# arbobendik/web-ray-tracer

Hardware: AMD Instinct MI355X
Metric: Mray/s at 1080p (spp x bounces x pixels / s) (higher is better)
Workload: dtype f32

## Files before the change

### web-ray-tracer_amd/csrc/flx_device.h

```cpp
#ifndef FLX_DEVICE_H
#define FLX_DEVICE_H

#include <hip/hip_runtime.h>
#include <stdint.h>

#include "flx_math.h"

#define FLX_DEV __device__ __forceinline__

namespace flx {

constexpr float PHI = 1.61803398874989484820459f;
constexpr float SQRT3 = 1.7320508075688772f;
constexpr float INV_PI = 0.3183098861837907f;
constexpr float INV_256 = 0.00390625f;
constexpr float INV_255 = 0.00392156862745098f;
constexpr float PI_F = 3.141592653589793f;
constexpr float BIAS = FLX_BIAS;
constexpr float POW32 = FLX_POW32;
constexpr float NEAR_VIEW_DEPTH = 0.5f;

struct f3 { float x, y, z; };
struct f4 { float x, y, z, w; };
struct M3 { f3 c0, c1, c2; };
// ... 555 lines not shown


FLX_DEV float divByRecip(float a, float d, float y) {
  float q = a * y;
  float r = __builtin_fmaf(-q, d, a);
  q = __builtin_fmaf(r, y, q);
  r = __builtin_fmaf(-q, d, a);
  return __builtin_fmaf(r, y, q);
}
FLX_DEV void reciprocalOfDir(const DeviceScene &sc, f3 d, f3 o, f3 &inv, bool &fast) {
  inv = F3(recipFast(d.x), recipFast(d.y), recipFast(d.z));
  const float LO = 8.673617379884035e-19f, HI = 1.152921504606847e18f, OHI = 5.764607523034235e17f;
  const float ax = flx_abs(d.x), ay = flx_abs(d.y), az = flx_abs(d.z);
  fast = sc.walk_fast_boxes != 0u && ax >= LO && ax <= HI && ay >= LO && ay <= HI && az >= LO && az <= HI &&
         flx_abs(o.x) <= OHI && flx_abs(o.y) <= OHI && flx_abs(o.z) <= OHI;
}
#ifndef FLX_WF_RECIP_DIV
#define FLX_WF_RECIP_DIV 1
#endif
FLX_DEV void walkPrepareRay(const DeviceScene &sc, WalkState &w) {
#if !FLX_WF_RECIP_DIV
  (void)sc; (void)w;
  return;
#endif
  reciprocalOfDir(sc, w.tR.dir, w.tR.origin, w.inv, w.fastDiv);
}
FLX_DEV bool rayCuboidRecip(float l, const WalkState &w, f3 minCorner, f3 maxCorner);
FLX_DEV bool rayCuboidR(float l, const WalkState &w, f3 minCorner, f3 maxCorner) {
#if !FLX_WF_RECIP_DIV
  return rayCuboid(l, w.tR, minCorner, maxCorner);
#else
  return rayCuboidRecip(l, w, minCorner, maxCorner);
#endif
}
FLX_DEV bool rayCuboidRecip(float l, const WalkState &w, f3 minCorner, f3 maxCorner) {
  const f3 o = w.tR.origin, d = w.tR.dir, y = w.inv;
  const f3 a0 = minCorner - o, a1 = maxCorner - o;
  uint32_t m = (flx_f2u(a0.x) << 1) - 2u;
  uint32_t t;
  t = (flx_f2u(a0.y) << 1) - 2u; m = t < m ? t : m;
  t = (flx_f2u(a0.z) << 1) - 2u; m = t < m ? t : m;
  t = (flx_f2u(a1.x) << 1) - 2u; m = t < m ? t : m;
  t = (flx_f2u(a1.y) << 1) - 2u; m = t < m ? t : m;
  t = (flx_f2u(a1.z) << 1) - 2u; m = t < m ? t : m;
  const bool aOk = m >= (0x2b800000u << 1) - 2u;
  f3 v0, v1;
  float tmin, tmax;
  if ((w.fastDiv && aOk)) {
    v0 = F3(divByRecip(a0.x, d.x, y.x), divByRecip(a0.y, d.y, y.y), divByRecip(a0.z, d.z, y.z));
    v1 = F3(divByRecip(a1.x, d.x, y.x), divByRecip(a1.y, d.y, y.y), divByRecip(a1.z, d.z, y.z));
    tmin = __builtin_fmaxf(__builtin_fmaxf(__builtin_fminf(v0.x, v1.x), __builtin_fminf(v0.y, v1.y)), __builtin_fminf(v0.z, v1.z));
    tmax = __builtin_fminf(__builtin_fminf(__builtin_fmaxf(v0.x, v1.x), __builtin_fmaxf(v0.y, v1.y)), __builtin_fmaxf(v0.z, v1.z));
    return tmax >= __builtin_fmaxf(tmin, BIAS) && tmin < l;
  }
  v0 = a0 / d;
  v1 = a1 / d;
  tmin = flx_max(flx_max(flx_min(v0.x, v1.x), flx_min(v0.y, v1.y)), flx_min(v0.z, v1.z));
  tmax = flx_min(flx_min(flx_max(v0.x, v1.x), flx_max(v0.y, v1.y)), flx_max(v0.z, v1.z));
  return tmax >= flx_max(tmin, BIAS) && tmin < l;
}

template <bool THICK = false> FLX_DEV bool rayCuboidFast(float l, const WalkState &w, f3 lo, f3 hi);
FLX_DEV Hit primaryWalkT(const DeviceScene &sc, const Ray &ray, float viewDepthPerS, uint32_t &visits) {
  Hit hit; hit.suv = F3(0.0f, 0.0f, 0.0f); hit.transformId = 0; hit.triangleId = -1;
  WalkState w;
  w.tR = ray; w.minLen = POW32;
  reciprocalOfDir(sc, ray.dir, ray.origin, w.inv, w.fastDiv);
  int cachedTI = 0;
  uint32_t link = sc.walk_root;
  while (link != WALK_END) {
    const size_t i = (size_t)linkIndex(link) * 3u;
    const float4 e0 = sc.walk[i], e1 = sc.walk[i + 1], e2 = sc.walk[i + 2];
    visits++;
    const int meta = __float_as_int(e2.z);
    if ((meta & 3) == 0) break;
    const int tI = (meta >> 2) << 1;
    if (tI != cachedTI) {
      const int iI = tI + 1;
      const M3 rotationII = rotation_at(sc, iI);
      cachedTI = tI;
      w.tR.origin = mul(rotationII, ray.origin + shift_at(sc, iI));
      w.tR.dir = mul(rotationII, ray.dir);
      reciprocalOfDir(sc, w.tR.dir, w.tR.origin, w.inv, w.fastDiv);
    }
    if ((meta & 3) == 1) {
      link = (uint32_t)__float_as_int(rayCuboidFast(w.minLen, w, F3(e0.x, e0.y, e0.z), F3(e0.w, e1.x, e1.y)) ? e2.x : e2.y);
    } else {
      f3 suv;
      if (moellerTrumborePrimaryE(F3(e0.x, e0.y, e0.z), F3(e0.w, e1.x, e1.y), F3(e1.z, e1.w, e2.x), w.tR, w.minLen, viewDepthPerS, suv)) {
        hit.suv = suv; hit.transformId = tI; hit.triangleId = __float_as_int(e2.w);
        w.minLen = suv.x;
      }
      link = (uint32_t)__float_as_int(e2.y);
    }
  }
  return hit;
}

typedef float flx_v4f_ __attribute__((ext_vector_type(4)));
extern "C" __device__ unsigned int __ockl_wfred_min_u32(unsigned int);
#ifndef FLX_PRIMARY_PREFETCH
#define FLX_PRIMARY_PREFETCH 0
#endif
#ifndef FLX_PRIMARY_LOCK_MIN
#define FLX_PRIMARY_LOCK_MIN 12
#endif
typedef __attribute__((address_space(4))) const flx_v4f_ fwd_cf4;
FLX_DEV void primaryVisit(const DeviceScene &sc, const Ray &ray, float viewDepthPerS, WalkState &w, int &cachedTI, Hit &hit, uint32_t &nxt,
                          float4 e0, float4 e1, float4 e2, int xfBase = 0 ) {
  const int meta = __float_as_int(e2.z);
  if ((meta & 3) == 0) { nxt = WALK_END; return; }
  const int tI = (meta >> 2) << 1;
  if (tI != cachedTI) {
    const int iI = tI + 1 + xfBase;
    const M3 rotationII = rotation_at(sc, iI);
    cachedTI = tI;
    w.tR.origin = mul(rotationII, ray.origin + shift_at(sc, iI));
    w.tR.dir = mul(rotationII, ray.dir);
    reciprocalOfDir(sc, w.tR.dir, w.tR.origin, w.inv, w.fastDiv);
  }
  if ((meta & 3) == 1) {
    nxt = (uint32_t)__float_as_int(rayCuboidFast(w.minLen, w, F3(e0.x, e0.y, e0.z), F3(e0.w, e1.x, e1.y)) ? e2.x : e2.y);
  } else {
    f3 suv;
    if (moellerTrumborePrimaryE(F3(e0.x, e0.y, e0.z), F3(e0.w, e1.x, e1.y), F3(e1.z, e1.w, e2.x), w.tR, w.minLen, viewDepthPerS, suv)) {
      hit.suv = suv; hit.transformId = tI; hit.triangleId = __float_as_int(e2.w);
      w.minLen = suv.x;
    }
    nxt = (uint32_t)__float_as_int(e2.y);
  }
}
FLX_DEV Hit primaryWalkF(const DeviceScene &sc, bool active, const Ray &ray, float viewDepthPerS, uint32_t &visits, int xfBase = 0) {
  Hit hit; hit.suv = F3(0.0f, 0.0f, 0.0f); hit.transformId = 0; hit.triangleId = -1;
  WalkState w;
  w.tR = ray; w.minLen = POW32;
  reciprocalOfDir(sc, ray.dir, ray.origin, w.inv, w.fastDiv);
  int cachedTI = 0;
  uint32_t nxt = active ? sc.fwd_root : WALK_END;
  const fwd_cf4 *L = (const fwd_cf4 *)sc.fwd;
  uint32_t thin = 0;
  for (;;) {
    const uint32_t i = __builtin_amdgcn_readfirstlane(__ockl_wfred_min_u32(nxt));
    if (i == WALK_END) return hit;
    uint32_t iu = i;
    asm volatile("" : "+s"(iu));
    const fwd_cf4 *E = L + (size_t)iu * 3u;
    const flx_v4f_ a = E[0], b = E[1], c = E[2];
    const bool mine = nxt == i;
    if (mine) {
      visits++;
      primaryVisit(sc, ray, viewDepthPerS, w, cachedTI, hit, nxt, make_float4(a.x, a.y, a.z, a.w), make_float4(b.x, b.y, b.z, b.w), make_float4(c.x, c.y, c.z, c.w), xfBase);
    }
    thin = (uint32_t)__popcll(flx_ballot(mine)) < (uint32_t)FLX_PRIMARY_LOCK_MIN ? thin + 1u : 0u;
    if (thin >= 2u) break;
  }
#if FLX_PRIMARY_PREFETCH
  if (nxt != WALK_END) {
    size_t i = (size_t)nxt * 3u;
    float4 e0 = sc.fwd[i], e1 = sc.fwd[i + 1], e2 = sc.fwd[i + 2];
    while (nxt != WALK_END) {
      const int meta = __float_as_int(e2.z);
      const bool box = (meta & 3) == 1;
      const uint32_t linkA = (uint32_t)__float_as_int(box ? e2.x : e2.y), linkB = (uint32_t)__float_as_int(e2.y);
      const size_t ia = (size_t)((meta & 3) == 0 || linkA == WALK_END ? 0u : linkA) * 3u, ib = (size_t)((meta & 3) == 0 || linkB == WALK_END ? 0u : linkB) * 3u;
      const float4 a0 = sc.fwd[ia], a1 = sc.fwd[ia + 1], a2 = sc.fwd[ia + 2];
      float4 b0 = a0, b1 = a1, b2 = a2;
      if (box) { b0 = sc.fwd[ib]; b1 = sc.fwd[ib + 1]; b2 = sc.fwd[ib + 2]; }
      visits++;
      primaryVisit(sc, ray, viewDepthPerS, w, cachedTI, hit, nxt, e0, e1, e2);
      const bool tookA = nxt == linkA;
      e0 = tookA ? a0 : b0; e1 = tookA ? a1 : b1; e2 = tookA ? a2 : b2;
    }
  }
#else
  while (nxt != WALK_END) {
    const size_t i = (size_t)nxt * 3u;
    const float4 e0 = sc.fwd[i], e1 = sc.fwd[i + 1], e2 = sc.fwd[i + 2];
    visits++;
    primaryVisit(sc, ray, viewDepthPerS, w, cachedTI, hit, nxt, e0, e1, e2, xfBase);
  }
#endif
  return hit;
}

template <bool COUNT>
FLX_DEV bool walkFetchT(const DeviceScene &sc, const float4 *lds, uint32_t ldsCount, WalkState &w, WalkEntry &cur, WorkCounters &cnt) {
  if ((uint32_t)w.i == WALK_END) return true;
  const uint32_t i = linkIndex((uint32_t)w.i);
  if (i < ldsCount) { cur.e0 = lds[3 * i]; cur.e1 = lds[3 * i + 1]; cur.e2 = lds[3 * i + 2]; }
  else { cur.e0 = sc.walk[3 * (size_t)i]; cur.e1 = sc.walk[3 * (size_t)i + 1]; cur.e2 = sc.walk[3 * (size_t)i + 2]; }
  if (COUNT) { if (w.mode == 0) cnt.shadow_visits++; else cnt.closest_visits++; }
  const int meta = __float_as_int(cur.e2.z);
  int tI = (meta >> 2) << 1;
  if (tI != w.cachedTI) {
    int iI = tI + 1;
    M3 rotationII = rotation_at(sc, iI);
    w.cachedTI = tI;
    w.tR.origin = mul(rotationII, w.src.origin + shift_at(sc, iI));
    f3 d = mul(rotationII, w.src.dir);
    w.tR.dir = (w.mode == 0) ? normalize(d) : d;
    walkPrepareRay(sc, w);
  }
  return (meta & 3) == 0;
}
FLX_DEV bool walkIsBoxT(const WalkEntry &cur) { return (__float_as_int(cur.e2.z) & 3) == 1; }
FLX_DEV bool walkIsBoxL(const WalkState &w) { return linkKind((uint32_t)w.i) == 1u; }
FLX_DEV void walkBoxT(WalkState &w, const WalkEntry &cur) {
  const bool hit = rayCuboidR(w.minLen, w, F3(cur.e0.x, cur.e0.y, cur.e0.z), F3(cur.e0.w, cur.e1.x, cur.e1.y));
  w.i = hit ? __float_as_int(cur.e2.x) : __float_as_int(cur.e2.y);
}
#ifndef FLX_MT_BRANCHFREE
#define FLX_MT_BRANCHFREE 1
#endif
FLX_DEV bool moellerTrumboreAny(f3 a, f3 edge1, f3 edge2, const Ray &ray, float l, bool cull, f3 &suv) {
  f3 pvec = cross(ray.dir, edge2);
  float det = dot(edge1, pvec);
  bool detBad = cull ? (det < BIAS) : (flx_abs(det) < BIAS);
  float inv_det = recipOfDet(det, detBad);
  f3 tvec = ray.origin - a;
  float u = dot(tvec, pvec) * inv_det;
  f3 qvec = cross(tvec, edge1);
  float v = dot(ray.dir, qvec) * inv_det;
  float uvSum = u + v;
  float s = dot(edge2, qvec) * inv_det;
  bool uBad = (u < BIAS) || (u > 1.0f);
  bool vBad = (v < BIAS) || (uvSum > 1.0f);
#if FLX_MT_BRANCHFREE
  const bool sLe = (s <= l) | (!cull & __builtin_isunordered(s, l));
  const bool sGt = (s > BIAS) | (!cull & (s != s));
  const bool sOk = sLe & sGt;
  suv = F3(s, u, v);
  return !detBad & !uBad & !vBad & sOk;
#else
  bool sOk = cull ? ((s <= l) && (s > BIAS)) : (!(s > l) && !(s <= BIAS));
  suv = F3(s, u, v);
  return !detBad && !uBad && !vBad && sOk;
#endif
}
#ifndef FLX_WF_LINK_XFORM
#define FLX_WF_LINK_XFORM 1
#endif
#ifndef FLX_WF_LINK_KIND
#define FLX_WF_LINK_KIND 1
#endif
#ifndef FLX_WF_LINK_ISBOX
#define FLX_WF_LINK_ISBOX 1
#endif
#ifndef FLX_WF_FLAT_FETCH
#define FLX_WF_FLAT_FETCH 1
#endif
FLX_DEV bool walkTriT(WalkState &w, const WalkEntry &cur) {
  f3 a = F3(cur.e0.x, cur.e0.y, cur.e0.z), edge1 = F3(cur.e0.w, cur.e1.x, cur.e1.y), edge2 = F3(cur.e1.z, cur.e1.w, cur.e2.x);
  f3 suv;
  const bool cull = w.mode == 0;
  const bool hit = moellerTrumboreAny(a, edge1, edge2, w.tR, w.minLen, cull, suv);
  bool ended = false;
  if ((hit)) {
    if (cull) { w.shadowed = true; ended = true; }
    else if (suv.x != 0.0f) {
      w.suv = suv; w.hitTI = (__float_as_int(cur.e2.z) >> 2) << 1; w.tri = __float_as_int(cur.e2.w);
      w.minLen = suv.x;
    }
  }
  w.i = __float_as_int(cur.e2.y);
  return ended;
}
FLX_DEV void walkStartT(const DeviceScene &sc, WalkState &w, int mode, const Ray &ray, float len) {
  w.mode = mode; w.src = ray; w.tR = ray; w.cachedTI = 0; w.minLen = len; w.i = (int)sc.walk_root;
  walkPrepareRay(sc, w);
}

FLX_DEV void walkSetupRays(const DeviceScene &sc, uint32_t nTransforms, const float4 *xf, float2 *rays, const Ray &src, bool shadowMode) {
  for (uint32_t t = 0; t < nTransforms; t++) {
    const float4 c0 = xf[4 * t], c1 = xf[4 * t + 1], c2 = xf[4 * t + 2], sh = xf[4 * t + 3];
    M3 rotationII; rotationII.c0 = F3(c0.x, c0.y, c0.z); rotationII.c1 = F3(c1.x, c1.y, c1.z); rotationII.c2 = F3(c2.x, c2.y, c2.z);
    f3 o = mul(rotationII, src.origin + F3(sh.x, sh.y, sh.z));
    f3 d = mul(rotationII, src.dir);
    if (flx_ballot(shadowMode) != 0ull) {
      f3 dn = normalize(d);
      if (shadowMode) d = dn;
    }
    f3 inv; bool fast;
    reciprocalOfDir(sc, d, o, inv, fast);
    rays[5 * t] = make_float2(o.x, o.y);
    rays[5 * t + 1] = make_float2(o.z, d.x);
    rays[5 * t + 2] = make_float2(d.y, d.z);
    rays[5 * t + 3] = make_float2(inv.x, inv.y);
    rays[5 * t + 4] = make_float2(inv.z, fast ? 1.0f : 0.0f);
  }
}
typedef float flx_v4f __attribute__((ext_vector_type(4)));
typedef float flx_v2f __attribute__((ext_vector_type(2)));
typedef __attribute__((address_space(3))) const flx_v4f lds_cf4;
typedef __attribute__((address_space(3))) const flx_v2f lds_cf2;
FLX_DEV float4 ldsLoad4(const lds_cf4 *p) { const flx_v4f v = *p; return make_float4(v.x, v.y, v.z, v.w); }
FLX_DEV void walkLoadRay(const float2 *raysGeneric, int t, WalkState &w) {
  const lds_cf2 *rays = (const lds_cf2 *)raysGeneric + __umul24((unsigned)t, 5u);
  const flx_v2f a = rays[0], b = rays[1], c = rays[2], d = rays[3], e = rays[4];
  w.tR.origin = F3(a.x, a.y, b.x);
  w.tR.dir = F3(b.y, c.x, c.y);
  w.inv = F3(d.x, d.y, e.x);
  w.fastDiv = e.y != 0.0f;
}
template <bool COUNT>
FLX_DEV bool walkFetchG(const float4 *walkG, const float4 *lds, uint32_t ldsCount, const float2 *rays, WalkState &w, WalkEntry &cur,
                        WorkCounters &cnt) {
#if FLX_WF_LINK_KIND
  const uint32_t link0 = (uint32_t)w.i;
  const bool stop = ((link0 + (1u << LINK_KIND_SHIFT)) & (2u << LINK_KIND_SHIFT)) == 0u;
#else
  if (COUNT) { if (((uint32_t)w.i == WALK_END)) return true; }
#endif
  const uint32_t i = linkIndex((uint32_t)w.i);
#if FLX_WF_FLAT_FETCH
  {
    const float4 *src = (i < ldsCount) ? lds + 3u * i : walkG + 3 * (size_t)i;
    cur.e0 = src[0]; cur.e1 = src[1]; cur.e2 = src[2];
  }
#else
  if (i < ldsCount) { const lds_cf4 *L = (const lds_cf4 *)lds + __umul24(i, 3u); cur.e0 = ldsLoad4(L); cur.e1 = ldsLoad4(L + 1); cur.e2 = ldsLoad4(L + 2); }
  else { cur.e0 = walkG[3 * (size_t)i]; cur.e1 = walkG[3 * (size_t)i + 1]; cur.e2 = walkG[3 * (size_t)i + 2]; }
#endif
#if FLX_WF_LINK_KIND
  if (COUNT) { if (linkKind(link0) != 3u) { if (w.mode == 0) cnt.shadow_visits++; else cnt.closest_visits++; } }
#else
  if (COUNT) { if (w.mode == 0) cnt.shadow_visits++; else cnt.closest_visits++; }
#endif
#if FLX_WF_LINK_XFORM
  if (FLX_UNLIKELY(((uint32_t)w.i & LINK_XFORM) != 0u)) {
    const int tI = (__float_as_int(cur.e2.z) >> 2) << 1;
    w.cachedTI = tI;
    walkLoadRay(rays, tI >> 1, w);
  }
#else
  const int tI = (__float_as_int(cur.e2.z) >> 2) << 1;
  if (FLX_UNLIKELY(tI != w.cachedTI)) {
    w.cachedTI = tI;
    walkLoadRay(rays, tI >> 1, w);
  }
#endif
#if FLX_WF_LINK_KIND
  return stop;
#else
  return (__float_as_int(cur.e2.z) & 3) == 0;
#endif
}
template <bool COUNT>
FLX_DEV bool walkFetchP(const DeviceScene &sc, const float4 *lds, uint32_t ldsCount, const float2 *rays, WalkState &w, WalkEntry &cur,
                        WorkCounters &cnt) {
  return walkFetchG<COUNT>(sc.walk, lds, ldsCount, rays, w, cur, cnt);
}
FLX_DEV const float4 *pinnedWalkCopy(const DeviceScene &sc) {
  const float4 *p = sc.walk;
  asm volatile("" : "+s"(p));
  return p;
}
FLX_DEV void walkLoadEntry(const DeviceScene &sc, const float4 *lds, uint32_t ldsCount, uint32_t i, WalkEntry &e) {
  if (i == WALK_END) { e.e0 = e.e1 = e.e2 = make_float4(0.f, 0.f, 0.f, 0.f); return; }
  i = linkIndex(i);
  if (i < ldsCount) { const lds_cf4 *L = (const lds_cf4 *)lds + __umul24(i, 3u); e.e0 = ldsLoad4(L); e.e1 = ldsLoad4(L + 1); e.e2 = ldsLoad4(L + 2); }
  else { e.e0 = sc.walk[3 * (size_t)i]; e.e1 = sc.walk[3 * (size_t)i + 1]; e.e2 = sc.walk[3 * (size_t)i + 2]; }
}
template <bool COUNT>
FLX_DEV bool walkArriveP(const float2 *rays, WalkState &w, const WalkEntry &cur, WorkCounters &cnt) {
  if ((uint32_t)w.i == WALK_END) return true;
  if (COUNT) { if (w.mode == 0) cnt.shadow_visits++; else cnt.closest_visits++; }
  const int meta = __float_as_int(cur.e2.z);
  const int tI = (meta >> 2) << 1;
  if (tI != w.cachedTI) {
    w.cachedTI = tI;
    walkLoadRay(rays, tI >> 1, w);
  }
  return (meta & 3) == 0;
}
#ifndef FLX_WF_BOX_INTERVAL
#define FLX_WF_BOX_INTERVAL 1
#endif
template <bool THICK = false>
FLX_DEV bool rayCuboidInterval(float l, const WalkState &w, f3 minCorner, f3 maxCorner, bool &sure) {
  const f3 o = w.tR.origin, y = w.inv;
  const float qx0 = (minCorner.x - o.x) * y.x, qx1 = (maxCorner.x - o.x) * y.x;
  const float qy0 = (minCorner.y - o.y) * y.y, qy1 = (maxCorner.y - o.y) * y.y;
  const float qz0 = (minCorner.z - o.z) * y.z, qz1 = (maxCorner.z - o.z) * y.z;
  const float nx = __builtin_fminf(qx0, qx1), fx = __builtin_fmaxf(qx0, qx1);
  const float ny = __builtin_fminf(qy0, qy1), fy = __builtin_fmaxf(qy0, qy1);
  const float nz = __builtin_fminf(qz0, qz1), fz = __builtin_fmaxf(qz0, qz1);
  constexpr float D = 4.76837158203125e-07f;
  const float nyz = __builtin_fmaxf(ny, nz), nxz = __builtin_fmaxf(nx, nz), nxy = __builtin_fmaxf(nx, ny);
  const float tmin = __builtin_fmaxf(nxy, nz), tmax = __builtin_fminf(__builtin_fminf(fx, fy), fz);
  const bool cx = THICK || __builtin_fmaf(-flx_abs(fx), D, fx) >= __builtin_fmaf(flx_abs(nyz), D, nyz);
  const bool cy = THICK || __builtin_fmaf(-flx_abs(fy), D, fy) >= __builtin_fmaf(flx_abs(nxz), D, nxz);
  const bool cz = THICK || __builtin_fmaf(-flx_abs(fz), D, fz) >= __builtin_fmaf(flx_abs(nxy), D, nxy);
  const float tminHi = __builtin_fmaf(flx_abs(tmin), D, tmin), tminLo = __builtin_fmaf(-flx_abs(tmin), D, tmin);
  const float tmaxHi = __builtin_fmaf(flx_abs(tmax), D, tmax), tmaxLo = __builtin_fmaf(-flx_abs(tmax), D, tmax);
  const bool sureTrue = (THICK ? tmaxLo >= tminHi : cx & cy & cz) & (tmaxLo >= BIAS) & (tminHi < l);
  const bool sureFalse = (tmaxHi < __builtin_fmaxf(tminLo, BIAS)) | (tminLo >= l);
  sure = w.fastDiv & (l >= 8.673617379884035e-19f) & (sureTrue | sureFalse);
  return sureTrue;
}
template <bool THICK>
FLX_DEV bool rayCuboidFast(float l, const WalkState &w, f3 lo, f3 hi) {
#if FLX_WF_BOX_INTERVAL
  bool sure;
  bool hit = rayCuboidInterval<THICK>(l, w, lo, hi, sure);
#if FLX_BOX_FALLBACK_COUNT
  w.boxTests++; if (!sure) w.boxExact++;
#endif
#ifndef FLX_BOX_UNSURE_BALLOT
#define FLX_BOX_UNSURE_BALLOT 0
#endif
#if FLX_BOX_UNSURE_BALLOT
  if (FLX_UNLIKELY(flx_ballot(!sure) != 0ull)) {
    if (!sure) hit = rayCuboidRecip(l, w, lo, hi);
  }
#else
  if (FLX_UNLIKELY(!sure)) hit = rayCuboidRecip(l, w, lo, hi);
#endif
  return hit;
#else
  return rayCuboidRecip(l, w, lo, hi);
#endif
}
template <bool THICK = false>
FLX_DEV void walkBoxP(WalkState &w, const WalkEntry &cur) {
  const bool hit = rayCuboidFast<THICK>(w.minLen, w, F3(cur.e0.x, cur.e0.y, cur.e0.z), F3(cur.e0.w, cur.e1.x, cur.e1.y));
  w.i = hit ? __float_as_int(cur.e2.x) : __float_as_int(cur.e2.y);
}

FLX_DEV bool nextBounceRuns(const DeviceFrame &fr, int i, f3 importancyFactor, f3 originalColor) {
  return (i + 1) < fr.max_reflections && length(importancyFactor * originalColor) >= fr.min_importancy * SQRT3;
}
typedef __attribute__((address_space(4))) const flx_v4f const_cf4;
template <bool COUNT, bool CULL>
FLX_DEV void walkLockPass(const DeviceScene &sc, bool active, const Ray &ray, float len, WalkState &w, uint32_t &visits) {
  w.tR = ray; w.minLen = len;
  reciprocalOfDir(sc, ray.dir, ray.origin, w.inv, w.fastDiv);
  uint32_t nxt = active ? sc.lock_root : WALK_END;
  const const_cf4 *L = (const const_cf4 *)sc.lock;
  const uint32_t n = sc.lock_entries;
  for (uint32_t i = 0; i < n; i++) {
    const bool mine = nxt == i;
    if (flx_ballot(mine) == 0ull) {
      if (flx_ballot(nxt != WALK_END) == 0ull) break;
      continue;
    }
    const const_cf4 *E = L + (size_t)__builtin_amdgcn_readfirstlane(i) * 3u;
    const flx_v4f e0 = E[0], e1 = E[1], e2 = E[2];
    const int meta = __float_as_int(e2.z);
    if (mine) {
      if (COUNT) visits++;
      if ((meta & 3) == 1) {
        const bool hit = rayCuboidFast(w.minLen, w, F3(e0.x, e0.y, e0.z), F3(e0.w, e1.x, e1.y));
        nxt = (uint32_t)__float_as_int(hit ? e2.x : e2.y);
      } else if ((meta & 3) == 2) {
        f3 suv;
        const bool hit = moellerTrumboreAny(F3(e0.x, e0.y, e0.z), F3(e0.w, e1.x, e1.y), F3(e1.z, e1.w, e2.x), w.tR, w.minLen, CULL, suv);
        nxt = (uint32_t)__float_as_int(e2.y);
        if (hit) {
          if (CULL) { w.shadowed = true; nxt = WALK_END; }
          else if (suv.x != 0.0f) {
            w.suv = suv; w.hitTI = (meta >> 2) << 1; w.tri = __float_as_int(e2.w);
            w.minLen = suv.x;
          }
        }
      } else {
        nxt = WALK_END;
      }
    }
  }
}

template <bool COUNT, bool LOCK>
FLX_DEV void walkBounce(const DeviceScene &sc, bool needShadow, bool needClosest, const Ray &shadowRay, float shadowLen, const Ray &nextRay,
                        bool &shadowed, Hit &hit, WorkCounters &cnt) {
  WalkState w;
  walkClearResults(w);
  if (LOCK) {
    w.cachedTI = 0;
    if (COUNT) { if (needShadow) cnt.shadow_walks++; if (needClosest) cnt.closest_walks++; }
    if (flx_ballot(needShadow) != 0ull) walkLockPass<COUNT, true>(sc, needShadow, shadowRay, shadowLen, w, cnt.shadow_visits);
    if (flx_ballot(needClosest) != 0ull) walkLockPass<COUNT, false>(sc, needClosest, nextRay, POW32, w, cnt.closest_visits);
    shadowed = w.shadowed;
    hit.suv = w.suv; hit.transformId = w.hitTI; hit.triangleId = w.tri;
    return;
  }
  if (!needShadow && !needClosest) {
    shadowed = false;
    hit.suv = w.suv; hit.transformId = w.hitTI; hit.triangleId = w.tri;
    return;
  }
  if (sc.n_transforms > 1u) {
    if (needShadow) walkStart(w, 0, shadowRay, shadowLen); else walkStart(w, 1, nextRay, POW32);
    if (COUNT) { if (needShadow) cnt.shadow_walks++; if (needClosest) cnt.closest_walks++; }
    while (w.mode != 2) {
      if (walkStep<COUNT>(sc, w, cnt)) {
        if (w.mode == 0 && needClosest) walkStart(w, 1, nextRay, POW32); else w.mode = 2;
      }
    }
    shadowed = w.shadowed;
    hit.suv = w.suv; hit.transformId = w.hitTI; hit.triangleId = w.tri;
    return;
  }
  w.mode = needShadow ? 0 : 1;
  w.src = needShadow ? shadowRay : nextRay;
  w.minLen = needShadow ? shadowLen : POW32;
  if (COUNT) { if (needShadow) cnt.shadow_walks++; if (needClosest) cnt.closest_walks++; }
  for (;;) {
    w.tR = w.src; w.cachedTI = 0;
    reciprocalOfDir(sc, w.tR.dir, w.tR.origin, w.inv, w.fastDiv);
    uint32_t link = sc.walk_root;
    for (;;) {
      if (((link + (1u << LINK_KIND_SHIFT)) & (2u << LINK_KIND_SHIFT)) == 0u) {
        if (COUNT) { if (linkKind(link) == 0u) { if (w.mode == 0) cnt.shadow_visits++; else cnt.closest_visits++; } }
        break;
      }
      const size_t i = (size_t)linkIndex(link) * 3u;
      WalkEntry cur;
      cur.e0 = sc.walk[i]; cur.e1 = sc.walk[i + 1]; cur.e2 = sc.walk[i + 2];
      if (COUNT) { if (w.mode == 0) cnt.shadow_visits++; else cnt.closest_visits++; }
      const bool isBox = linkKind(link) == 1u;
      if (FLX_UNLIKELY((link & LINK_XFORM) != 0u)) {
        const int tI = (__float_as_int(cur.e2.z) >> 2) << 1;
        const int iI = tI + 1;
        const M3 rotationII = rotation_at(sc, iI);
        w.cachedTI = tI;
        w.tR.origin = mul(rotationII, w.src.origin + shift_at(sc, iI));
        const f3 d = mul(rotationII, w.src.dir);
        w.tR.dir = (w.mode == 0) ? normalize(d) : d;
        reciprocalOfDir(sc, w.tR.dir, w.tR.origin, w.inv, w.fastDiv);
      }
      if (isBox) {
        walkBoxP(w, cur);
        link = (uint32_t)w.i;
      } else {
        const bool ended = walkTriT(w, cur);
        link = ended ? WALK_END : (uint32_t)w.i;
      }
    }
    if (w.mode == 0 && needClosest) { w.mode = 1; w.src = nextRay; w.minLen = POW32; continue; }
    break;
  }
  shadowed = w.shadowed;
  hit.suv = w.suv; hit.transformId = w.hitTI; hit.triangleId = w.tri;
}

FLX_DEV void bounceFinish(PixelState &ps, PathState &p, const ShadeOut &so, bool shadowedByWalk) {
  bool shadowed = so.shadowedNoWalk || (so.needShadow && shadowedByWalk);
  if (shadowed && so.markId) ps.renderId.w += INV_255;
  f3 localColor = shadowed ? so.baseLuminance : so.litColor;
  p.finalColor = p.finalColor + localColor * p.importancyFactor;
}

template <bool COUNT, bool LOCK>
FLX_DEV bool bounceOn(const DeviceScene &sc, const DeviceFrame &fr, const SurfaceCtx &sf, PixelState &ps, PathState &p, f3 camera, float cosSampleN,
                      int i, WorkCounters &cnt) {
  ShadeOut so;
  shadeSample(sc, fr, sf, ps, p, camera, cosSampleN, i, so);
  bool shadowed;
  walkBounce<COUNT, LOCK>(sc, so.needShadow, nextBounceRuns(fr, i, p.importancyFactor, ps.originalColor), so.shadowRay, so.shadowLen, p.ray, shadowed, p.hit, cnt);
  bounceFinish(ps, p, so, shadowed);
  if (p.hit.triangleId == -1) return false;
  p.lastHitPoint = p.ray.origin;
  return true;
}

template <bool COUNT, bool LOCK>
FLX_DEV bool bounce(const DeviceScene &sc, const DeviceFrame &fr, PixelState &ps, PathState &p, f3 camera, float cosSampleN, int i,
                    WorkCounters &cnt) {
  ShadeOut so;
  bounceShade<COUNT>(sc, fr, ps, p, camera, cosSampleN, i, so, cnt);
  bool shadowed;
  walkBounce<COUNT, LOCK>(sc, so.needShadow, nextBounceRuns(fr, i, p.importancyFactor, ps.originalColor), so.shadowRay, so.shadowLen, p.ray, shadowed, p.hit, cnt);
  bounceFinish(ps, p, so, shadowed);
  if (p.hit.triangleId == -1) return false;
  p.lastHitPoint = p.ray.origin;
  return true;
}

FLX_DEV f3 primary_dir_v(const DeviceFrame &fr, const FrameView &v, uint32_t px, uint32_t py_gl, float &nx, float &ny, float &viewDepthPerS) {
  nx = ((float)px + 0.5f) / (float)fr.width * 2.0f - 1.0f;
  ny = ((float)py_gl + 0.5f) / (float)fr.height * 2.0f - 1.0f;
  const float *iv = v.inv_view;
  f3 d = F3((iv[0] * nx + iv[1] * ny) + iv[2], (iv[3] * nx + iv[4] * ny) + iv[5], (iv[6] * nx + iv[7] * ny) + iv[8]);
  d = normalize(d);
  viewDepthPerS = dot(F3(v.view_row2[0], v.view_row2[1], v.view_row2[2]), d);
  return d;
}
FLX_DEV f3 primary_dir(const DeviceFrame &fr, uint32_t f, uint32_t px, uint32_t py_gl, float &nx, float &ny, float &viewDepthPerS) {
  return primary_dir_v(fr, fr.view[f], px, py_gl, nx, ny, viewDepthPerS);
}

}
#endif
```

### web-ray-tracer_amd/csrc/flx_frame_common.h

```cpp
#pragma once
#include "flx_kernels.h"
#include "flx_kernel_util.h"
#include "flx_wavefront_common.h"

namespace flx {

#ifndef FLX_WF_WALK_THREADS
#define FLX_WF_WALK_THREADS 1024
#endif
#ifndef FLX_WF_WAVES_PER_EU
#define FLX_WF_WAVES_PER_EU 4
#endif
#ifndef FLX_WF_LDS_TOTAL
#define FLX_WF_LDS_TOTAL (156 * 1024)
#endif
#ifndef FLX_WF_INNER
#define FLX_WF_INNER 8
#endif
#ifndef FLX_WF_UNROLL
#define FLX_WF_UNROLL 8
#endif
#ifndef FLX_WF_BATCH
#define FLX_WF_BATCH 24
#endif
#ifndef FLX_WF_DRAWS_PER_WAVE
#define FLX_WF_DRAWS_PER_WAVE 16
#endif
#ifndef FLX_FRAME_SHADERS_FRONT
#define FLX_FRAME_SHADERS_FRONT 3
#endif
#ifndef FLX_FRAME_PROLOGUE_WAVES
#define FLX_FRAME_PROLOGUE_WAVES 2
#endif
#ifndef FLX_FRAME_READY_UNITS
#define FLX_FRAME_READY_UNITS 32
#endif

typedef const __attribute__((address_space(4))) FrameArgs *FrameArgsP;
FLX_DEV const FrameArgs &frame_args(FrameArgsP p) { asm volatile("" : "+s"(p)); return *(const FrameArgs *)p; }
FLX_DEV FrameArgsP kernel_frame_args() { return (FrameArgsP)__builtin_amdgcn_kernarg_segment_ptr(); }
#define FLX_ARGS_OF(ab) const FrameArgs &A_ = frame_args(ab); const DeviceScene &sc = A_.sc; const DeviceFrame &fr = A_.fr; const WavefrontBuffers &wb = A_.wb; (void)sc; (void)fr; (void)wb

template <bool VER>
FLX_DEV uint32_t scene_version_of(const DeviceFrame &fr, uint32_t frameIdx) { return VER ? blockIdx.x * fr.frames + frameIdx : 0u; }

template <bool COUNT, bool LV = false, bool VER = false>
FLX_DEV bool shade0_tile(FrameArgsP ab, uint32_t tile, uint32_t lane, float4 h, WorkCounters &cnt, const FrameView *lv = nullptr) {
  uint32_t S, frameIdx, lightBase = 0;
  int tri;
  bool alive, compact;
  f3 camera;
  SurfaceCtx sf;
  float ndcX = 0.0f, ndcY = 0.0f;
  Hit hit;
  {
  FLX_ARGS_OF(ab);
  S = (uint32_t)fr.samples;
  uint32_t px, k;
  tile8_pixel(fr, tile, lane, px, k);
  const bool inFrame = px < fr.width && k < fr.rows;
  frameIdx = inFrame ? frame_index(fr, k) : 0u;
  camera = view_camera(view_at<LV>(fr, lv, frameIdx));
  tri = inFrame ? __float_as_int(h.w) : -1;
  alive = tri != -1 && fr.max_reflections > 0 && length(F3(1.0f, 1.0f, 1.0f) * F3(1.0f, 1.0f, 1.0f)) >= fr.min_importancy * SQRT3;
  hit.suv = F3(h.x, h.y, h.z); hit.triangleId = tri; hit.transformId = 0;
  compact = wb.rec0 != nullptr;
  if (alive) {
    hit.transformId = (int)sc.geometry[3 * tri + 2].y << 1;
    if (VER) { const uint32_t ver = scene_version_of<VER>(fr, frameIdx); hit.transformId += (int)(ver * 2u * sc.n_transforms); lightBase = ver * 6u * sc.n_lights; }
    const uint32_t py_gl = fr.height - 1u - image_row(fr, k);
    float viewDepthPerS;
    Ray pr;
    pr.origin = camera;
    pr.dir = primary_dir_v(fr, view_at<LV>(fr, lv, frameIdx), px, py_gl, ndcX, ndcY, viewDepthPerS);
    const WorkCounters before = cnt;
    shadeSurface<COUNT>(sc, fr, hit, pr, camera, sf, cnt);
    if (COUNT) {
      cnt.shades = before.shades + (cnt.shades - before.shades) * S;
      cnt.atlas_texels = before.atlas_texels + (cnt.atlas_texels - before.atlas_texels) * S;
    }
  }
  }
  for (uint32_t s = 0; s < S; s++) {
    FLX_ARGS_OF(ab);
    const uint32_t pathId = ((tile * S + s) << 6) | lane;
    float4 *rec = wb.rec + (size_t)pathId * 8;
    if (!alive) {
      if (tri != -1) finalize_path<LV>(fr, wb, pathId, F3(0.0f, 0.0f, 0.0f), F3(1.0f, 1.0f, 1.0f), F3(1.0f, 1.0f, 1.0f), lv);
      if (compact) wb.rec0[(size_t)pathId * 3] = make_float4(0.f, 0.f, 0.f, __int_as_float(RF_DEAD));
      else rec[0] = make_float4(0.f, 0.f, 0.f, __int_as_float(RF_DEAD));
      continue;
    }
    PathState p;
    PixelState ps;
    ps.firstRayLength = 1.0f; ps.glassFilter = 0.0f; ps.originalRMEx = 0.0f; ps.originalTPOx = 0.0f;
    ps.renderId.x = ps.renderId.y = ps.renderId.z = ps.renderId.w = 0.0f;
    ps.renderOriginalId = ps.renderId;
    ps.ndc_x = ndcX; ps.ndc_y = ndcY;
    ps.seed = view_at<LV>(fr, lv, frameIdx).random_seed;
    ps.lightBase = lightBase;
    ps.originalColor = F3(1.0f, 1.0f, 1.0f);
    p.hit = hit;
    p.lastHitPoint = camera;
    p.dontFilter = true;
    p.importancyFactor = F3(1.0f, 1.0f, 1.0f);
    const float cosSampleN = flx_cos((float)s);
    ShadeOut so;
    shadeSample(sc, fr, sf, ps, p, camera, cosSampleN, 0, so);
    const int flags = (p.dontFilter ? RF_DONT_FILTER : 0) | (so.needShadow ? RF_NEED_SHADOW : 0) | (so.shadowedNoWalk ? RF_SHADOWED_NO_WALK : 0) |
                      (nextBounceRuns(fr, 0, p.importancyFactor, ps.originalColor) ? 0 : RF_NO_CLOSEST);
    if (compact) {
      if (s == 0u) {
        float4 *pp = wb.pix0 + (((size_t)tile << 6) | lane) * 3;
        pp[0] = make_float4(p.ray.origin.x, p.ray.origin.y, p.ray.origin.z, 0.0f);
        pp[1] = make_float4(so.shadowRay.origin.x, so.shadowRay.origin.y, so.shadowRay.origin.z, 0.0f);
        pp[2] = make_float4(ps.originalColor.x, ps.originalColor.y, ps.originalColor.z, so.baseLuminance.x);
      }
      float4 *r0 = wb.rec0 + (size_t)pathId * 3;
      r0[0] = make_float4(p.ray.dir.x, p.ray.dir.y, p.ray.dir.z, __int_as_float(flags));
      r0[1] = make_float4(so.shadowRay.dir.x, so.shadowRay.dir.y, so.shadowRay.dir.z, so.shadowLen);
      r0[2] = make_float4(so.litColor.x, so.litColor.y, so.litColor.z, 0.0f);
      continue;
    }
    rec[0] = make_float4(p.ray.origin.x, p.ray.origin.y, p.ray.origin.z, __int_as_float(flags));
    rec[1] = make_float4(p.ray.dir.x, p.ray.dir.y, p.ray.dir.z, so.shadowLen);
    rec[2] = make_float4(so.shadowRay.origin.x, so.shadowRay.origin.y, so.shadowRay.origin.z, so.baseLuminance.x);
    rec[3] = make_float4(so.shadowRay.dir.x, so.shadowRay.dir.y, so.shadowRay.dir.z, __int_as_float(0));
    rec[4] = make_float4(so.litColor.x, so.litColor.y, so.litColor.z, 0.0f);
    rec[5] = make_float4(0.0f, 0.0f, 0.0f, 0.0f);
    rec[6] = make_float4(p.importancyFactor.x, p.importancyFactor.y, p.importancyFactor.z, 0.0f);
    rec[7] = make_float4(ps.originalColor.x, ps.originalColor.y, ps.originalColor.z, 0.0f);
  }
  return alive;
}

template <bool COUNT, bool LV = false, bool VER = false>
FLX_DEV float4 primary_tile(FrameArgsP ab, uint32_t tile, uint32_t lane, WorkCounters &cnt, const FrameView *lv = nullptr) {
  FLX_ARGS_OF(ab);
  float4 *__restrict__ hits = const_cast<float4 *>(wb.hits);
  uint32_t px, k;
  tile8_pixel(fr, tile, lane, px, k);
  const bool inImage = px < fr.width && k < fr.rows;
  float nx, ny, viewDepthPerS = 0.0f;
  Ray pr; pr.origin = F3(0.0f, 0.0f, 0.0f); pr.dir = F3(0.0f, 0.0f, 1.0f);
  int xfBase = 0;
  if (inImage) {
    const uint32_t py_gl = fr.height - 1u - image_row(fr, k);
    const uint32_t frameIdx = frame_index(fr, k);
    if (VER) xfBase = (int)(scene_version_of<VER>(fr, frameIdx) * 2u * sc.n_transforms);
    const FrameView &v = view_at<LV>(fr, lv, frameIdx);
    pr.dir = primary_dir_v(fr, v, px, py_gl, nx, ny, viewDepthPerS);
    pr.origin = view_camera(v);
  }
  const uint32_t visitsBefore = cnt.primary_visits;
  const Hit hp = primaryWalkF(sc, inImage, pr, viewDepthPerS, cnt.primary_visits, xfBase);
  if (COUNT && wb.tileCost && wb.tileCostPrimary) {
    const uint32_t nTiles = ((fr.width + 7u) >> 3) * ((fr.rows + 7u) >> 3);
    atomicAdd(wb.tileCost + nTiles + tile, (unsigned long long)(cnt.primary_visits - visitsBefore));
  }
  float4 h = make_float4(hp.suv.x, hp.suv.y, hp.suv.z, __int_as_float(inImage ? hp.triangleId : -1));
  if (inImage) {
    if (COUNT && hp.triangleId != -1) cnt.primary_hits++;
    hits[(size_t)k * fr.width + px] = h;
  }
  return h;
}

template <bool COUNT, bool LV = false, bool VER = false>
FLX_DEV void shade_path(FrameArgsP ab, uint32_t pathId, WorkCounters &cnt, const FrameView *lv = nullptr) {
  FLX_ARGS_OF(ab);
  float4 *rec = wb.rec + (size_t)pathId * 8;
  uint32_t px, k, s;
  item_pixel(fr, pathId, px, k, s);
  const uint32_t frameIdx = frame_index(fr, k);
  const f3 camera = view_camera(view_at<LV>(fr, lv, frameIdx));
  PathState p;
  PixelState ps;
  ps.firstRayLength = 1.0f; ps.glassFilter = 0.0f; ps.originalRMEx = 0.0f; ps.originalTPOx = 0.0f;
  ps.renderId.x = ps.renderId.y = ps.renderId.z = ps.renderId.w = 0.0f;
  ps.renderOriginalId = ps.renderId;
  const float4 q0 = rec[0], q1 = rec[1], q2 = rec[2], q3 = rec[3], q6 = rec[6], q7 = rec[7];
  const int pb = __float_as_int(q3.w) + 1;
  p.ray.origin = F3(q0.x, q0.y, q0.z);
  p.lastHitPoint = p.ray.origin;
  p.ray.dir = F3(q1.x, q1.y, q1.z);
  p.hit.suv = F3(q2.x, q2.y, q2.z);
  p.hit.triangleId = __float_as_int(q2.w);
  p.hit.transformId = (int)sc.geometry[3 * p.hit.triangleId + 2].y << 1;
  if (VER) { const uint32_t ver = scene_version_of<VER>(fr, frameIdx); p.hit.transformId += (int)(ver * 2u * sc.n_transforms); ps.lightBase = ver * 6u * sc.n_lights; }
  p.dontFilter = (__float_as_int(q0.w) & RF_DONT_FILTER) != 0;
  p.importancyFactor = F3(q6.x, q6.y, q6.z);
  ps.originalColor = F3(q7.x, q7.y, q7.z);
  const uint32_t py_gl = fr.height - 1u - image_row(fr, k);
  float viewDepthPerS;
  (void)primary_dir_v(fr, view_at<LV>(fr, lv, frameIdx), px, py_gl, ps.ndc_x, ps.ndc_y, viewDepthPerS);
  ps.seed = view_at<LV>(fr, lv, frameIdx).random_seed;
  const float cosSampleN = flx_cos((float)s);
  ShadeOut so;
  bounceShade<COUNT>(sc, fr, ps, p, camera, cosSampleN, pb, so, cnt);
  const int flags = (p.dontFilter ? RF_DONT_FILTER : 0) | (so.needShadow ? RF_NEED_SHADOW : 0) | (so.shadowedNoWalk ? RF_SHADOWED_NO_WALK : 0) |
                    (nextBounceRuns(fr, pb, p.importancyFactor, ps.originalColor) ? 0 : RF_NO_CLOSEST);
  rec[0] = make_float4(p.ray.origin.x, p.ray.origin.y, p.ray.origin.z, __int_as_float(flags));
  rec[1] = make_float4(p.ray.dir.x, p.ray.dir.y, p.ray.dir.z, so.shadowLen);
  rec[2] = make_float4(so.shadowRay.origin.x, so.shadowRay.origin.y, so.shadowRay.origin.z, so.baseLuminance.x);
  rec[3] = make_float4(so.shadowRay.dir.x, so.shadowRay.dir.y, so.shadowRay.dir.z, __int_as_float(pb));
  rec[4] = make_float4(so.litColor.x, so.litColor.y, so.litColor.z, 0.0f);
  rec[6] = make_float4(p.importancyFactor.x, p.importancyFactor.y, p.importancyFactor.z, 0.0f);
  rec[7] = make_float4(ps.originalColor.x, ps.originalColor.y, ps.originalColor.z, 0.0f);
}

struct WalkLane {
  int st;
  uint32_t pathId; int flags; int pathBounce; float base;
  Ray nextRay, shadowRay; float shadowLen;
  WalkState w; WalkEntry cur;
  uint32_t v0;
};
FLX_DEV void walkLaneInit(WalkLane &L) {
  L.v0 = 0u;
  L.st = P_EMPTY; L.pathId = 0; L.flags = 0; L.pathBounce = 0; L.base = 0.0f;
  L.nextRay.origin = F3(0.f, 0.f, 0.f); L.nextRay.dir = L.nextRay.origin;
  L.shadowRay = L.nextRay; L.shadowLen = 0.0f;
  walkClearResults(L.w);
  L.w.src = L.nextRay; L.w.tR = L.nextRay; L.w.minLen = 0.0f; L.w.i = 0; L.w.cachedTI = 0;
  L.w.mode = 2;
  L.cur.e0 = L.cur.e1 = L.cur.e2 = make_float4(0.f, 0.f, 0.f, 0.f);
}
FLX_DEV const float4 *pix_part(const DeviceFrame &fr, const WavefrontBuffers &wb, uint32_t id) {
  uint32_t tile0, s0;
  item_tile(fr, id, tile0, s0);
  return wb.pix0 + (((size_t)tile0 << 6) | (id & 63u)) * 3;
}
#define FLX_WALK_LANE_FOLD(LV_, fr_, wb_, compactRecs_, L_, lv_, toShade_, ended_, costed_, stamp_)                              \
  do {                                                                                                                           \
    float4 *rec_ = (wb_).rec + (size_t)(L_).pathId * 8;                                                                          \
    const bool compact_ = (compactRecs_) && (L_).pathBounce == 0;                                                                \
    float4 q4_, q5_, q6_, q7_;                                                                                                   \
    const float4 *pp_ = nullptr;                                                                                                 \
    if (compact_) {                                                                                                              \
      pp_ = pix_part(fr_, wb_, (L_).pathId);                                                                                     \
      q4_ = (wb_).rec0[(size_t)(L_).pathId * 3 + 2]; q7_ = pp_[2];                                                               \
      q5_ = make_float4(0.0f, 0.0f, 0.0f, 0.0f); q6_ = make_float4(1.0f, 1.0f, 1.0f, 0.0f);                                      \
    } else {                                                                                                                     \
      q4_ = rec_[4]; q5_ = rec_[5]; q6_ = rec_[6]; q7_ = rec_[7];                                                                \
    }                                                                                                                            \
    const bool shadowed_ = ((L_).flags & RF_SHADOWED_NO_WALK) || (((L_).flags & RF_NEED_SHADOW) && (L_).w.shadowed);            \
    const f3 localColor_ = shadowed_ ? F3((L_).base, (L_).base, (L_).base) : F3(q4_.x, q4_.y, q4_.z);                            \
    const f3 importancy_ = F3(q6_.x, q6_.y, q6_.z), originalColor_ = F3(q7_.x, q7_.y, q7_.z);                                    \
    const f3 finalColor_ = F3(q5_.x, q5_.y, q5_.z) + localColor_ * importancy_;                                                  \
     \
    const float cost_ = (costed_) ? q5_.w + (float)(((stamp_) - ((uint32_t)(L_).flags >> 8)) & 0xffffffu) : 1.0f;      \
    bool cont_ = (L_).w.tri != -1;                                                                                               \
    if (cont_) cont_ = ((L_).pathBounce + 1) < (fr_).max_reflections && length(importancy_ * originalColor_) >= (fr_).min_importancy * SQRT3;      \
    if (cont_) {                                                                                                                 \
      if (compact_) {                                         \
        const float4 a_ = (wb_).rec0[(size_t)(L_).pathId * 3], bq_ = (wb_).rec0[(size_t)(L_).pathId * 3 + 1], p0_ = pp_[0];      \
        rec_[0] = make_float4(p0_.x, p0_.y, p0_.z, a_.w);                                                                        \
        rec_[1] = make_float4(a_.x, a_.y, a_.z, bq_.w);                                                                          \
        rec_[3] = make_float4(bq_.x, bq_.y, bq_.z, __int_as_float(0));                                                           \
        rec_[6] = make_float4(1.0f, 1.0f, 1.0f, 0.0f);                                                                           \
        rec_[7] = make_float4(q7_.x, q7_.y, q7_.z, 0.0f);                                                                        \
      }                                                                                                                          \
      rec_[5] = make_float4(finalColor_.x, finalColor_.y, finalColor_.z, (costed_) ? cost_ : 0.0f);                                                 \
      rec_[2] = make_float4((L_).w.suv.x, (L_).w.suv.y, (L_).w.suv.z, __int_as_float((L_).w.tri));                               \
      toShade_ = true;                                                                                                           \
    } else {                                                                                                                     \
      finalize_path<LV_>(fr_, wb_, (L_).pathId, finalColor_, importancy_, originalColor_, lv_, cost_);                           \
      ended_ = true;                                                                                                             \
    }                                                                                                                            \
    (L_).st = P_EMPTY;                                                                                                           \
  } while (0)

struct WalkRecord { float4 q0, q1, q2, q3; };
FLX_DEV void walkLaneFetchRecord(const DeviceFrame &fr, const WavefrontBuffers &wb, uint32_t id, bool compactFresh, WalkRecord &R) {
  const float4 *rec = wb.rec + (size_t)id * 8;
  if (compactFresh) {
    const float4 *pp = pix_part(fr, wb, id);
    const float4 a = wb.rec0[(size_t)id * 3], bq = wb.rec0[(size_t)id * 3 + 1];
    const float4 p0 = pp[0], p1 = pp[1], p2 = pp[2];
    R.q0 = make_float4(p0.x, p0.y, p0.z, a.w);
    R.q1 = make_float4(a.x, a.y, a.z, bq.w);
    R.q2 = make_float4(p1.x, p1.y, p1.z, p2.w);
    R.q3 = make_float4(bq.x, bq.y, bq.z, __int_as_float(0));
  } else {
    R.q0 = rec[0]; R.q1 = rec[1]; R.q2 = rec[2]; R.q3 = rec[3];
  }
}
template <bool COUNT>
FLX_DEV bool walkLaneInstall(uint32_t id, const WalkRecord &R, WalkLane &L, WorkCounters &cnt, uint32_t stamp = 0u ) {
  const int fl = __float_as_int(R.q0.w);
  if (fl & RF_DEAD) return true;
  L.pathId = id; L.flags = fl | (int)(stamp << 8); L.base = R.q2.w; L.pathBounce = __float_as_int(R.q3.w);
  L.nextRay.origin = F3(R.q0.x, R.q0.y, R.q0.z);
  L.nextRay.dir = F3(R.q1.x, R.q1.y, R.q1.z);
  L.shadowRay.origin = F3(R.q2.x, R.q2.y, R.q2.z);
  L.shadowRay.dir = F3(R.q3.x, R.q3.y, R.q3.z);
  L.shadowLen = R.q1.w;
  walkClearResults(L.w);
  L.w.mode = (fl & RF_NEED_SHADOW) ? 0 : 1;
  if (COUNT) { if (L.w.mode == 0) cnt.shadow_walks++; if (!(fl & RF_NO_CLOSEST)) cnt.closest_walks++; L.v0 = cnt.closest_visits + cnt.shadow_visits; }
  L.st = (L.w.mode == 1 && (fl & RF_NO_CLOSEST)) ? P_DONE : P_SETUP;
  return false;
}
template <bool COUNT>
FLX_DEV bool walkLaneLoad(const DeviceFrame &fr, const WavefrontBuffers &wb, uint32_t id, bool compactFresh, WalkLane &L, WorkCounters &cnt, uint32_t stamp = 0u) {
  WalkRecord R;
  walkLaneFetchRecord(fr, wb, id, compactFresh, R);
  return walkLaneInstall<COUNT>(id, R, L, cnt, stamp);
}
template <bool COUNT>
FLX_DEV void walkLaneSetup(const DeviceScene &sc, uint32_t nTransforms, const float4 *xf, float2 *myRays, const float4 *walkG, const float4 *ldsEntries, uint32_t ldsCount,
                           WalkLane &L, WorkCounters &cnt) {
  const bool shadowMode = L.w.mode == 0;
  const Ray src = shadowMode ? L.shadowRay : L.nextRay;
  walkSetupRays(sc, nTransforms, xf, myRays, src, shadowMode);
  L.w.tR = src; L.w.cachedTI = 0; L.w.minLen = shadowMode ? L.shadowLen : POW32; L.w.i = (int)sc.walk_root;
  reciprocalOfDir(sc, src.dir, src.origin, L.w.inv, L.w.fastDiv);
  L.st = P_WALKING;
  if (walkFetchG<COUNT>(walkG, ldsEntries, ldsCount, myRays, L.w, L.cur, cnt)) L.st = shadowMode ? P_SWITCH : P_DONE;
}
FLX_DEV void walkLaneSwitch(WalkLane &L) {
  if (L.st == P_SWITCH) {
    if (L.flags & RF_NO_CLOSEST) L.st = P_DONE;
    else { L.w.mode = 1; L.st = P_SETUP; }
  }
}
#define FLX_WALK_LANE_STEP(COUNT_, THICK_, walkG_, ldsEntries_, ldsCount_, myRays_, L_, cnt_)                                      \
  do {                                                                                                                           \
    if ((L_).st == P_WALKING) {                                                                                                  \
      bool ended_ = false;                                                                                                       \
      if (FLX_WF_LINK_ISBOX ? walkIsBoxL((L_).w) : walkIsBoxT((L_).cur)) walkBoxP<THICK_>((L_).w, (L_).cur); else ended_ = walkTriT((L_).w, (L_).cur);                             \
      if (!ended_) ended_ = walkFetchG<COUNT_>(walkG_, ldsEntries_, ldsCount_, myRays_, (L_).w, (L_).cur, cnt_);                 \
      if (ended_) (L_).st = ((L_).w.mode == 0) ? P_SWITCH : P_DONE;                                                              \
    }                                                                                                                            \
  } while (0)

constexpr uint32_t FQ_SIZE = WF_FRAME_RING;
#ifndef FLX_FQ_LIMIT
#define FLX_FQ_LIMIT 4096
#endif
constexpr uint32_t FQ_LIMIT = FLX_FQ_LIMIT;
constexpr uint32_t FQ_ALIVE_MAX = FQ_SIZE - 256u;
#ifndef FLX_FQ_WATCHDOG_LOG2
#define FLX_FQ_WATCHDOG_LOG2 24
#endif
constexpr uint32_t FQ_WATCHDOG = 1u << FLX_FQ_WATCHDOG_LOG2;
enum { FC_ALIVE = 0, FC_DRY = 1, FC_SQ = 2 , FC_WQ = 5 , FC_RQ = 8 , FC_FRONT_DONE = 11, FC_WORDS = 16 };
#ifndef FLX_FRAME_READY_UNITS
#define FLX_FRAME_READY_UNITS 32
#endif

FLX_DEV uint32_t fq_load(uint32_t *p) { return __hip_atomic_load(p, __ATOMIC_RELAXED, __HIP_MEMORY_SCOPE_WORKGROUP); }
FLX_DEV void fq_push(uint32_t *ring, uint32_t *ctl, bool mine, uint32_t id, uint32_t lane) {
  const unsigned long long m = flx_ballot(mine);
  if (m == 0ull) return;
  const uint32_t c = (uint32_t)__popcll(m);
  uint32_t pos0 = 0;
  if (lane == 0) pos0 = atomicAdd(&ctl[0], c);
  pos0 = __builtin_amdgcn_readfirstlane(pos0);
  if (mine) __hip_atomic_store(&ring[(pos0 + lane_rank(m)) & (FQ_SIZE - 1u)], id, __ATOMIC_RELAXED, __HIP_MEMORY_SCOPE_WORKGROUP);
  __builtin_amdgcn_fence(__ATOMIC_RELEASE, "workgroup");
  if (lane == 0) atomicAdd(&ctl[2], c);
}
FLX_DEV uint32_t fq_pop(uint32_t *ring, uint32_t *ctl, unsigned long long takers, uint32_t want, uint32_t atLeast, uint32_t lane, uint32_t &id) {
  uint32_t n = 0, pos0 = 0;
  if (lane == 0) {
    uint32_t a = fq_load(&ctl[2]);
    while (a != 0u && a >= atLeast) {
      const uint32_t take = a < want ? a : want;
      const uint32_t seen = atomicCAS(&ctl[2], a, a - take);
      if (seen == a) { n = take; pos0 = atomicAdd(&ctl[1], take); break; }
      a = seen;
    }
  }
  n = __builtin_amdgcn_readfirstlane(n);
  pos0 = __builtin_amdgcn_readfirstlane(pos0);
  if (n == 0u) return 0u;
  const uint32_t r = lane_rank(takers);
  if (((takers >> lane) & 1ull) != 0ull && r < n) {
    uint32_t *slot = &ring[(pos0 + r) & (FQ_SIZE - 1u)];
    uint32_t v, spins = 0;
    do { v = fq_load(slot); } while (v == WF_INVALID && ++spins < FQ_WATCHDOG);
    __hip_atomic_store(slot, WF_INVALID, __ATOMIC_RELAXED, __HIP_MEMORY_SCOPE_WORKGROUP);
    id = v;
  }
  __builtin_amdgcn_fence(__ATOMIC_ACQUIRE, "workgroup");
  return n;
}


}
```

Baseline: 11860.

## Issue next walk-entry fetch before triangle test to overlap load latency

Splits the BVH walk fetch into an issue phase and an arrival phase. In the lane step, the next entry's load is issued before the triangle intersection runs, using the link stored in the current entry, so memory/LDS latency overlaps with triangle math. This relies on the link-kind and link-isbox encodings so that control flow does not wait on the loaded data. It adds register pressure, since a second WalkEntry stays live, and uses undefined-value asm placeholders for inactive lanes.

```diff
diff --git a/web-ray-tracer_amd/csrc/flx_device.h b/web-ray-tracer_amd/csrc/flx_device.h
--- a/web-ray-tracer_amd/csrc/flx_device.h
+++ b/web-ray-tracer_amd/csrc/flx_device.h
@@ -881,48 +881,54 @@
   w.inv = F3(d.x, d.y, e.x);
   w.fastDiv = e.y != 0.0f;
 }
+FLX_DEV void walkFetchIssue(const float4 *walkG, const float4 *lds, uint32_t ldsCount, uint32_t link, WalkEntry &e) {
+  const uint32_t i = linkIndex(link);
+#if FLX_WF_FLAT_FETCH
+  {
+    const float4 *src = (i < ldsCount) ? lds + 3u * i : walkG + 3 * (size_t)i;
+    e.e0 = src[0]; e.e1 = src[1]; e.e2 = src[2];
+  }
+#else
+  if (i < ldsCount) { const lds_cf4 *L = (const lds_cf4 *)lds + __umul24(i, 3u); e.e0 = ldsLoad4(L); e.e1 = ldsLoad4(L + 1); e.e2 = ldsLoad4(L + 2); }
+  else { e.e0 = walkG[3 * (size_t)i]; e.e1 = walkG[3 * (size_t)i + 1]; e.e2 = walkG[3 * (size_t)i + 2]; }
+#endif
+}
+template <bool COUNT>
+FLX_DEV bool walkFetchArrive(const float2 *rays, WalkState &w, const WalkEntry &e, WorkCounters &cnt) {
+#if FLX_WF_LINK_KIND
+  const uint32_t link0 = (uint32_t)w.i;
+  const bool stop = ((link0 + (1u << LINK_KIND_SHIFT)) & (2u << LINK_KIND_SHIFT)) == 0u;
+  if (COUNT) { if (linkKind(link0) != 3u) { if (w.mode == 0) cnt.shadow_visits++; else cnt.closest_visits++; } }
+#else
+  if (COUNT) { if (w.mode == 0) cnt.shadow_visits++; else cnt.closest_visits++; }
+#endif
+#if FLX_WF_LINK_XFORM
+  if (FLX_UNLIKELY(((uint32_t)w.i & LINK_XFORM) != 0u)) {
+    const int tI = (__float_as_int(e.e2.z) >> 2) << 1;
+    w.cachedTI = tI;
+    walkLoadRay(rays, tI >> 1, w);
+  }
+#else
+  const int tI = (__float_as_int(e.e2.z) >> 2) << 1;
+  if (FLX_UNLIKELY(tI != w.cachedTI)) {
+    w.cachedTI = tI;
+    walkLoadRay(rays, tI >> 1, w);
+  }
+#endif
+#if FLX_WF_LINK_KIND
+  return stop;
+#else
+  return (__float_as_int(e.e2.z) & 3) == 0;
+#endif
+}
 template <bool COUNT>
 FLX_DEV bool walkFetchG(const float4 *walkG, const float4 *lds, uint32_t ldsCount, const float2 *rays, WalkState &w, WalkEntry &cur,
                         WorkCounters &cnt) {
-#if FLX_WF_LINK_KIND
-  const uint32_t link0 = (uint32_t)w.i;
-  const bool stop = ((link0 + (1u << LINK_KIND_SHIFT)) & (2u << LINK_KIND_SHIFT)) == 0u;
-#else
+#if !FLX_WF_LINK_KIND
   if (COUNT) { if (((uint32_t)w.i == WALK_END)) return true; }
 #endif
-  const uint32_t i = linkIndex((uint32_t)w.i);
-#if FLX_WF_FLAT_FETCH
-  {
-    const float4 *src = (i < ldsCount) ? lds + 3u * i : walkG + 3 * (size_t)i;
-    cur.e0 = src[0]; cur.e1 = src[1]; cur.e2 = src[2];
-  }
-#else
-  if (i < ldsCount) { const lds_cf4 *L = (const lds_cf4 *)lds + __umul24(i, 3u); cur.e0 = ldsLoad4(L); cur.e1 = ldsLoad4(L + 1); cur.e2 = ldsLoad4(L + 2); }
-  else { cur.e0 = walkG[3 * (size_t)i]; cur.e1 = walkG[3 * (size_t)i + 1]; cur.e2 = walkG[3 * (size_t)i + 2]; }
-#endif
-#if FLX_WF_LINK_KIND
-  if (COUNT) { if (linkKind(link0) != 3u) { if (w.mode == 0) cnt.shadow_visits++; else cnt.closest_visits++; } }
-#else
-  if (COUNT) { if (w.mode == 0) cnt.shadow_visits++; else cnt.closest_visits++; }
-#endif
-#if FLX_WF_LINK_XFORM
-  if (FLX_UNLIKELY(((uint32_t)w.i & LINK_XFORM) != 0u)) {
-    const int tI = (__float_as_int(cur.e2.z) >> 2) << 1;
-    w.cachedTI = tI;
-    walkLoadRay(rays, tI >> 1, w);
-  }
-#else
-  const int tI = (__float_as_int(cur.e2.z) >> 2) << 1;
-  if (FLX_UNLIKELY(tI != w.cachedTI)) {
-    w.cachedTI = tI;
-    walkLoadRay(rays, tI >> 1, w);
-  }
-#endif
-#if FLX_WF_LINK_KIND
-  return stop;
-#else
-  return (__float_as_int(cur.e2.z) & 3) == 0;
-#endif
+  walkFetchIssue(walkG, lds, ldsCount, (uint32_t)w.i, cur);
+  return walkFetchArrive<COUNT>(rays, w, cur, cnt);
 }
 template <bool COUNT>
 FLX_DEV bool walkFetchP(const DeviceScene &sc, const float4 *lds, uint32_t ldsCount, const float2 *rays, WalkState &w, WalkEntry &cur,
diff --git a/web-ray-tracer_amd/csrc/flx_frame_common.h b/web-ray-tracer_amd/csrc/flx_frame_common.h
--- a/web-ray-tracer_amd/csrc/flx_frame_common.h
+++ b/web-ray-tracer_amd/csrc/flx_frame_common.h
@@ -325,6 +325,35 @@
     else { L.w.mode = 1; L.st = P_SETUP; }
   }
 }
+#ifndef FLX_WF_TRI_EARLY_FETCH
+#define FLX_WF_TRI_EARLY_FETCH 1
+#endif
+#if FLX_WF_TRI_EARLY_FETCH && !(FLX_WF_LINK_KIND && FLX_WF_LINK_ISBOX)
+#error "FLX_WF_TRI_EARLY_FETCH needs FLX_WF_LINK_KIND and FLX_WF_LINK_ISBOX: neither the arrival nor the trip's control may wait for the loaded entry"
+#endif
+FLX_DEV float4 walkAnyFloat4() {
+  float x, y, z, w;
+  asm volatile("" : "=v"(x)); asm volatile("" : "=v"(y)); asm volatile("" : "=v"(z)); asm volatile("" : "=v"(w));
+  return make_float4(x, y, z, w);
+}
+#if FLX_WF_TRI_EARLY_FETCH
+#define FLX_WALK_LANE_STEP(COUNT_, THICK_, walkG_, ldsEntries_, ldsCount_, myRays_, L_, cnt_)                                      \
+  do {                                                                                                                           \
+    WalkEntry nxt_;                                                                                                              \
+    nxt_.e0 = walkAnyFloat4(); nxt_.e1 = walkAnyFloat4(); nxt_.e2 = walkAnyFloat4();                                             \
+    if ((L_).st == P_WALKING) {                                                                                                  \
+      bool ended_ = false;                                                                                                       \
+      uint32_t here_ = (uint32_t)(L_).w.i;                                        \
+      if (walkIsBoxL((L_).w)) walkBoxP<THICK_>((L_).w, (L_).cur); else (L_).w.i = __float_as_int((L_).cur.e2.y);                 \
+      walkFetchIssue(walkG_, ldsEntries_, ldsCount_, (uint32_t)(L_).w.i, nxt_);                                                  \
+      asm("" : "+v"(here_));                                                                                                     \
+      if (linkKind(here_) != 1u) ended_ = walkTriT((L_).w, (L_).cur);                                                            \
+      if (!ended_) ended_ = walkFetchArrive<COUNT_>(myRays_, (L_).w, nxt_, cnt_);                                                \
+      if (ended_) (L_).st = ((L_).w.mode == 0) ? P_SWITCH : P_DONE;                                                              \
+    }                                                                                                                            \
+    (L_).cur = nxt_;                                                                                                             \
+  } while (0)
+#else
 #define FLX_WALK_LANE_STEP(COUNT_, THICK_, walkG_, ldsEntries_, ldsCount_, myRays_, L_, cnt_)                                      \
   do {                                                                                                                           \
     if ((L_).st == P_WALKING) {                                                                                                  \
@@ -334,6 +363,7 @@
       if (ended_) (L_).st = ((L_).w.mode == 0) ? P_SWITCH : P_DONE;                                                              \
     }                                                                                                                            \
   } while (0)
+#endif
 
 constexpr uint32_t FQ_SIZE = WF_FRAME_RING;
 #ifndef FLX_FQ_LIMIT
```

Result: faster. 12430 (median of 6 runs) (+4.8%).
